# nanoporetech/taiyaki

Measured on AMD Instinct MI355X. Metric: signal-chunks/sec (T=4000) flip-flop train step, higher is better.
Workload: dtype f32; 1 GPU; configs[1]: mLstm_flipflop r9.4.1 DNA, chunk_len=4000 (T=800 blocks), 128 chunks/GPU, size 256, HIP flip-flop CRF loss + logZ, gradient maxima/clipping, AdamW; config_id=2, model=mLstm_flipflop, global_batch=128, chunk_len=4000, launch=hipGraph replay of forward+loss and of AdamW, eager backward, hw_queues=4, conv=gemm, lstm=miopen, batches=pre-assembled, cycled from HBM, parallelism=dp1 (reads sharded; one flat RCCL gradient all-reduce after backward)

## Files before the change

taiyaki_amd/csrc/lstm_kernels.hip:

```cpp
#include "dispatch.h"
#include "ff_common.h"
#include "lstm_bwd_layout.h"
#include "rnn_common.h"

namespace tk {
namespace {

template <int U>
constexpr int threads_for() { return U == 48 ? 384 : U <= 32 ? 256 : 512; }
template <int H, int U>
constexpr int bwd_threads_for() { return U == 48 ? 2 * H : threads_for<U>(); }

template <int H, int C, int U, bool VL = false, bool SAVE = !VL>
__global__ __launch_bounds__(threads_for<U>(), 1) void lstm_fwd_kernel(const float *__restrict__ gx,
                                                                       const float *__restrict__ whh, int T, Cols cols,
                                                                       int reverse, int ngroups,
                                                                       float *__restrict__ y,
                                                                       float *__restrict__ gates,
                                                                       float *__restrict__ cell, u64 *hbuf,
                                                                       uint32_t *status,
                                                                       const int32_t *__restrict__ lengths) {
    constexpr int NT = threads_for<U>();
    const int N = cols.n, LD = cols.ld();
    constexpr int G = H / U;
    constexpr int KP = NT / U;
    constexpr int KS = H / KP;
    constexpr int NG = (H * C + NT - 1) / NT;
    static_assert(KS >= 1 && KP <= 64 && C <= KP, "lane (u, kp) inside one wave; one cell lane per (u, column)");
    constexpr int U4 = U / 4;
    constexpr int NQ = SAVE ? (6 * C * U4 + NT - 1) / NT : 1;
    static_assert(U % 4 == 0, "a row of the staging block is whole 16-byte chunks");
    __shared__ __attribute__((aligned(16))) float hs[2][H * C];
    __shared__ __attribute__((aligned(16))) float stg[SAVE ? 2 : 1][SAVE ? 6 * C * U : 4];
    __shared__ int give_up;

    int group, member;
    place(G, group, member);
    const int tid = threadIdx.x;
    const int j0 = member * U, n0 = group * C;
    const int u = tid / KP, kp = tid % KP;

    float w[4][KS];
#pragma unroll
    for (int g = 0; g < 4; ++g)
#pragma unroll
        for (int i = 0; i < KS; ++i) w[g][i] = whh[((size_t)g * H + j0 + u) * H + i * KP + kp];
    settle(w);

    int col = 0;
#pragma unroll
    for (int m = 1, width = C; width > 1; m <<= 1, width >>= 1)
        if (kp & m) col += width / 2;
    const bool cell_lane = kp < C;
    const int n = n0 + col;
    const bool valid = cell_lane && n < N;
    float cst = 0.f;
    int len = 0;
    if constexpr (VL) len = !valid ? 0 : lengths ? lengths[n] : T;

    for (int i = tid; i < H * C; i += NT) hs[0][i] = 0.f;
    if (tid == 0) give_up = 0;

    const size_t H4 = 4 * (size_t)H;
    float *rp[NQ];
    size_t rpitch[NQ];
    if constexpr (SAVE) {
#pragma unroll
        for (int i = 0; i < NQ; ++i) {
            const int q = tid + i * NT, row = q / U4, v = row / C, nn = n0 + row % C;
            const size_t w = v < 2 ? (size_t)H : H4;
            float *base = v == 0 ? y : v == 1 ? cell : gates + (size_t)(v - 2) * H;
            rpitch[i] = (size_t)LD * w;
            rp[i] = q < 6 * C * U4 && nn < N ? base + (size_t)nn * w + j0 + 4 * (q % U4) : nullptr;
        }
    }
    float gq[4] = {0.f, 0.f, 0.f, 0.f};
    if (valid) {
        const float *p = gx + ((size_t)(reverse ? T - 1 : 0) * LD + n) * H4 + j0 + u;
#pragma unroll
        for (int g = 0; g < 4; ++g) gq[g] = p[(size_t)g * H];
    }
    float held = 0.f;
    __syncthreads();

    for (int s = 0; s < T; ++s) {
        const int t = reverse ? T - 1 - s : s;
        float *hb = hs[s & 1];
        settle(gq);
        if (s > 0) {
            const u64 *src = hbuf + ((size_t)((s - 1) & 1) * ngroups + group) * (H * C);
            float v[NG];
            if (!sweep<NG>(src, tid, NT, H * C, (unsigned)s, v, status)) give_up = 1;
#pragma unroll
            for (int q = 0; q < NG; ++q) {
                const int e = tid + q * NT;
                if (e < H * C) hb[(e % H) * C + e / H] = v[q];
            }
            __syncthreads();
            if (give_up) return;
            const int tl = reverse ? t + 1 : t - 1;
            if constexpr (!SAVE) {
                if (valid) y[((size_t)tl * LD + n) * H + j0 + u] = held;
            } else {
                rows_to_global<NQ>(stg[(s - 1) & 1], tid, NT, rp, rpitch, (size_t)tl);
            }
        }
        float gn[4] = {0.f, 0.f, 0.f, 0.f};
        if (valid && s + 1 < T) {
            const float *p = gx + ((size_t)(reverse ? t - 1 : t + 1) * LD + n) * H4 + j0 + u;
#pragma unroll
            for (int g = 0; g < 4; ++g) gn[g] = p[(size_t)g * H];
        }
        asm volatile("" ::: "memory");

        float acc[4][C];
#pragma unroll
        for (int g = 0; g < 4; ++g)
#pragma unroll
            for (int c = 0; c < C; ++c) acc[g][c] = 0.f;
#pragma unroll
        for (int i = 0; i < KS; ++i) {
            float hv[C];
            lds_row<C>(hb + (i * KP + kp) * C, hv);
#pragma unroll
            for (int g = 0; g < 4; ++g)
#pragma unroll
                for (int c = 0; c < C; ++c) acc[g][c] = fmaf(w[g][i], hv[c], acc[g][c]);
        }
#pragma unroll
        for (int m = 1; m < KP; m <<= 1) {
            const int half = C / (2 * m);
            const bool up = (kp & m) != 0;
#pragma unroll
            for (int g = 0; g < 4; ++g) {
                if (half == 0) acc[g][0] += __shfl_xor(acc[g][0], m);
#pragma unroll
                for (int c = 0; c < C / 2; ++c) {
                    if (c < half) {
                        const float send = up ? acc[g][c] : acc[g][c + half];
                        const float keep = up ? acc[g][c + half] : acc[g][c];
                        acc[g][c] = keep + __shfl_xor(send, m);
                    }
                }
            }
        }

        if (cell_lane) {
            float ig = sigmoidf(acc[0][0] + gq[0]), fg = sigmoidf(acc[1][0] + gq[1]);
            float gg = tanhf(acc[2][0] + gq[2]), og = sigmoidf(acc[3][0] + gq[3]);
            cst = fmaf(ig, gg, fg * cst);
            float h = og * tanhf(cst);
            if constexpr (VL) {
                if (t >= len) {
                    cst = h = 0.f;
                    if constexpr (SAVE) ig = fg = gg = og = 0.f;
                }
            }
            if (s + 1 < T)
                store_granule(hbuf + ((size_t)(s & 1) * ngroups + group) * (H * C) + col * H + j0 + u,
                              (unsigned)(s + 1), h);
            if constexpr (!SAVE) {
                held = h;
            } else {
                float *sp = stg[s & 1] + col * U + u;
                sp[0 * C * U] = h;
                sp[1 * C * U] = cst;
                sp[2 * C * U] = ig;
                sp[3 * C * U] = fg;
                sp[4 * C * U] = gg;
                sp[5 * C * U] = og;
            }
        }
#pragma unroll
        for (int g = 0; g < 4; ++g) gq[g] = gn[g];
    }
    if (T > 0) {
        const int tl = reverse ? 0 : T - 1;
        if constexpr (!SAVE) {
            if (valid) y[((size_t)tl * LD + n) * H + j0 + u] = held;
        } else {
            __syncthreads();
            rows_to_global<NQ>(stg[(T - 1) & 1], tid, NT, rp, rpitch, (size_t)tl);
        }
    }
}

#ifndef TK_RNN_VARLEN
template <int M>
__device__ __forceinline__ float xor_lane(float v) {
    static_assert(M == 1 || M == 2 || M == 4, "a partner inside the lane's group of 8");
    const int x = __float_as_int(v);
    if constexpr (M == 1) {
        return __int_as_float(__builtin_amdgcn_update_dpp(0, x, 0xB1, 0xF, 0xF, true));
    } else if constexpr (M == 2) {
        return __int_as_float(__builtin_amdgcn_update_dpp(0, x, 0x4E, 0xF, 0xF, true));
    } else {
        const int y = __builtin_amdgcn_update_dpp(0, x, 0x141, 0xF, 0xF, true);
        return __int_as_float(__builtin_amdgcn_update_dpp(0, y, 0x1B, 0xF, 0xF, true));
    }
}

template <int M, int RQ, int NA>
__device__ __forceinline__ void halve_rounds(float (&acc)[NA], int rq) {
    if constexpr (M < RQ) {
        constexpr int n = NA / (2 * M);
        const bool up = (rq & M) != 0;
#pragma unroll
        for (int a = 0; a < n; ++a) {
            const float send = up ? acc[a] : acc[a + n];
            const float keep = up ? acc[a + n] : acc[a];
            acc[a] = keep + xor_lane<M>(send);
        }
        halve_rounds<2 * M, RQ>(acc, rq);
    }
}

template <int H, int C, int U, bool VL = false>
__global__ __launch_bounds__((bwd_threads_for<H, U>()), 1) void lstm_bwd_kernel(const float *__restrict__ whh,
                                                                       const float *__restrict__ gates,
                                                                       const float *__restrict__ cell,
                                                                       const float *__restrict__ dy, int T, Cols cols,
                                                                       int reverse, int ngroups,
                                                                       float *__restrict__ dgates, u64 *pbuf,
                                                                       uint32_t *status,
                                                                       const int32_t *__restrict__ lengths) {
    constexpr int NT = bwd_threads_for<H, U>();
    const int N = cols.n, LD = cols.ld();
    constexpr int G = H / U;
    constexpr bool STRIDED = U == 48;
    constexpr int RP = NT / H;
    constexpr int R = 4 * U / RP;
    constexpr LstmBwdBlock LB(NT, H, U, C);
    constexpr bool BLOCK = LB.KQ > 0;
    constexpr int KQ = BLOCK ? LB.KQ : 1, RQ = BLOCK ? LB.RQ : 1, RR = BLOCK ? LB.RR : 1, KEEP = BLOCK ? LB.KEEP : 1;
    constexpr int PAIRS = U * C;
    constexpr int PL = NT / PAIRS;
    constexpr int NP = (G + PL - 1) / PL;
    constexpr bool APART = BLOCK && NP > 1;
    static_assert(!APART || NP * PL == G, "every plane polls NP producers");
    static_assert(RP >= 1 && R >= 1 && PL >= 1 && PL * PAIRS == NT, "every lane polls; one cell lane per pair");
    static_assert(!STRIDED || (RP * H == NT && R * RP == 4 * U && U % RP == 0),
                  "a lane's rows keep their gate index at compile time");
    static_assert(!BLOCK || (LB.ok() && KQ * RR * NT == 4 * U * H && RQ <= 64 && (RQ & (RQ - 1)) == 0 &&
                             KEEP * NT == C * H && KQ * RR == R),
                  "every owned weight in one lane; the RQ partial sums inside one wave; one granule per held sum");
    __shared__ __attribute__((aligned(16))) float dgs[4 * U * C];
    __shared__ float gath[(APART ? G : PL) * PAIRS];
    __shared__ __attribute__((aligned(16))) float red[RP > 1 && !BLOCK ? RP * C * H : 1];
    __shared__ int give_up;

    int group, member;
    place(G, group, member);
    const int tid = threadIdx.x;
    const int j0 = member * U, n0 = group * C;

    const int k = tid % H, rp = tid / H;
    const int kb = tid / RQ, rq = tid % RQ;
    float w[R];
    if constexpr (BLOCK) {
#pragma unroll
        for (int j = 0; j < RR; ++j) {
            const int r = LB.row(rq, j);
#pragma unroll
            for (int q = 0; q < KQ; ++q) w[q * RR + j] = whh[((size_t)(r / U) * H + j0 + (r % U)) * H + KQ * kb + q];
        }
    } else if constexpr (STRIDED) {
        const float *wbase = whh + (size_t)(j0 + rp) * H + k;
#pragma unroll
        for (int i = 0; i < R; ++i) w[i] = wbase[(unsigned)((((i * RP) / U) * H + (i * RP) % U) * H)];
    } else {
#pragma unroll
        for (int i = 0; i < R; ++i) {
            const int r = rp * R + i;
            w[i] = whh[((size_t)(r / U) * H + j0 + (r % U)) * H + k];
        }
    }
    settle(w);

    const bool cell_lane = tid < PAIRS;
    const int pair = tid % PAIRS, plane = tid / PAIRS;
    const int cc = pair / U, u = pair % U;
    const int n = n0 + cc;
    const bool valid = cell_lane && n < N;
    float dc_next = 0.f, f_next = 0.f;
    int len = 0;
    if constexpr (VL) len = !valid ? 0 : lengths ? lengths[n] : T;
    if (tid == 0) give_up = 0;

    const size_t H4 = 4 * (size_t)H;
    float in[7] = {0.f, 0.f, 0.f, 0.f, 0.f, 0.f, 0.f};
    if (valid) {
        const int t = reverse ? 0 : T - 1;
        const size_t o = ((size_t)t * LD + n) * H + j0 + u;
        in[0] = dy[o];
        in[1] = cell[o];
        if (T > 1) in[2] = cell[((size_t)(reverse ? t + 1 : t - 1) * LD + n) * H + j0 + u];
        const float *gp = gates + ((size_t)t * LD + n) * H4 + j0 + u;
#pragma unroll
        for (int g = 0; g < 4; ++g) in[3 + g] = gp[(size_t)g * H];
    }
    float held[4] = {0.f, 0.f, 0.f, 0.f};
    __syncthreads();

    const u64 *mine = pbuf + (size_t)group * G * C * H + cc * H + j0 + u;
    const int a0 = LB.kept_first(rq), pub = (a0 % C) * H + KQ * kb + a0 / C;
    for (int s = 0; s < T; ++s) {
        const int tt = T - 1 - s;
        const int t = reverse ? T - 1 - tt : tt;
        const int tp = reverse ? t + 1 : t - 1;
        settle(in);
        float dhr = 0.f;
        if (s > 0) {
            float v[NP];
            const int nvalid = plane < G ? (G - plane + PL - 1) / PL : 0;
            const u64 *src = mine + (size_t)((s - 1) & 1) * ngroups * G * C * H;
            if (!sweep<NP>(src, plane * C * H, PL * C * H, G * C * H, (unsigned)s, v, status)) give_up = 1;
            if constexpr (APART) {
#pragma unroll
                for (int q = 0; q < NP; ++q) gath[(plane + q * PL) * PAIRS + pair] = v[q];
            } else {
                float sum = 0.f;
#pragma unroll
                for (int q = 0; q < NP; ++q)
                    if (q < nvalid) sum += v[q];
                gath[plane * PAIRS + pair] = sum;
            }
            __syncthreads();
            if (give_up) return;
            if (cell_lane) {
#pragma unroll
                for (int p = 0; p < (APART ? G : PL); ++p) dhr += gath[p * PAIRS + pair];
            }
            if (valid) {
                const int tl = reverse ? t - 1 : t + 1;
                float *dp = dgates + ((size_t)tl * LD + n) * H4 + j0 + u;
#pragma unroll
                for (int g = 0; g < 4; ++g) dp[(size_t)g * H] = held[g];
            }
        }
        float nx[7] = {0.f, 0.f, 0.f, 0.f, 0.f, 0.f, 0.f};
        if (valid && tt > 0) {
            const size_t o = ((size_t)tp * LD + n) * H + j0 + u;
            nx[0] = dy[o];
            nx[1] = in[2];
            if (tt > 1) nx[2] = cell[((size_t)(reverse ? tp + 1 : tp - 1) * LD + n) * H + j0 + u];
            const float *gp = gates + ((size_t)tp * LD + n) * H4 + j0 + u;
#pragma unroll
            for (int g = 0; g < 4; ++g) nx[3 + g] = gp[(size_t)g * H];
        }
        asm volatile("" ::: "memory");

        if (cell_lane) {
            const float ct = in[1];
            float cp = in[2];
            if constexpr (VL) {
                if (tp >= len) cp = 0.f;
            }
            const float ig = in[3], gg = in[5], og = in[6];
            float fg = in[4];
            const float dh = in[0] + dhr;
            const float tc = tanhf(ct);
            float dc = dh * og * (1.f - tc * tc) + dc_next * f_next;
            float di = dc * gg * ig * (1.f - ig);
            float df = dc * cp * fg * (1.f - fg);
            float dg = dc * ig * (1.f - gg * gg);
            float dout = dh * tc * og * (1.f - og);
            if constexpr (VL) {
                if (t >= len) dc = fg = di = df = dg = dout = 0.f;
            }
            dc_next = dc;
            f_next = fg;
            held[0] = di;
            held[1] = df;
            held[2] = dg;
            held[3] = dout;
            dgs[(0 * U + u) * C + cc] = valid ? di : 0.f;
            dgs[(1 * U + u) * C + cc] = valid ? df : 0.f;
            dgs[(2 * U + u) * C + cc] = valid ? dg : 0.f;
            dgs[(3 * U + u) * C + cc] = valid ? dout : 0.f;
        }
#pragma unroll
        for (int q = 0; q < 7; ++q) in[q] = nx[q];
        __syncthreads();
        if (s + 1 == T) break;

        if constexpr (BLOCK) {
            u64 *dst = pbuf + (((size_t)(s & 1) * ngroups + group) * G + member) * C * H;
            float acc[KQ * C];
#pragma unroll
            for (int a = 0; a < KQ * C; ++a) acc[a] = 0.f;
#pragma unroll
            for (int i = 0; i < RR / 2; ++i) {
                float d[2 * C];
                lds_row<2 * C>(dgs + (rq + RQ * i) * 2 * C, d);
#pragma unroll
                for (int e = 0; e < 2; ++e)
#pragma unroll
                    for (int q = 0; q < KQ; ++q)
#pragma unroll
                        for (int c = 0; c < C; ++c)
                            acc[q * C + c] = fmaf(w[q * RR + 2 * i + e], d[e * C + c], acc[q * C + c]);
            }
            halve_rounds<1, RQ>(acc, rq);
#pragma unroll
            for (int v = 0; v < KEEP; ++v) store_granule(dst + pub + v * H, (unsigned)(s + 1), acc[v]);
            continue;
        }
        float acc[C];
#pragma unroll
        for (int c = 0; c < C; ++c) acc[c] = 0.f;
#pragma unroll
        for (int i = 0; i < R; ++i) {
            float d[C];
            lds_row<C>(dgs + (STRIDED ? i * RP + rp : rp * R + i) * C, d);
#pragma unroll
            for (int c = 0; c < C; ++c) acc[c] = fmaf(w[i], d[c], acc[c]);
        }
        u64 *dst = pbuf + (((size_t)(s & 1) * ngroups + group) * G + member) * C * H;
        if constexpr (RP == 1) {
#pragma unroll
            for (int c = 0; c < C; ++c) store_granule(dst + c * H + k, (unsigned)(s + 1), acc[c]);
        } else {
#pragma unroll
            for (int c = 0; c < C; ++c) red[(rp * C + c) * H + k] = acc[c];
            __syncthreads();
            for (int e = tid; e < C * H; e += NT) {
                float v = 0.f;
#pragma unroll
                for (int q = 0; q < RP; ++q) v += red[q * C * H + e];
                store_granule(dst + e, (unsigned)(s + 1), v);
            }
        }
    }
    if (valid && T > 0) {
        const int tl = reverse ? T - 1 : 0;
        float *dp = dgates + ((size_t)tl * LD + n) * H4 + j0 + u;
#pragma unroll
        for (int g = 0; g < 4; ++g) dp[(size_t)g * H] = held[g];
    }
}

#endif

int g_lab_cols = 0;
int g_lab_units = 0;

int units48(size_t H) { return H == 192 || H == 384 ? 48 : 0; }

bool lstm_geometry(size_t N, size_t H, int cu_count, int *C_out, int *groups_out) {
    const int U48 = units48(H);
    if (!(U48 || H == 16 || H == 32 || H == 64 || H == 128 || H == 256) || N == 0 || cu_count <= 0) return false;
    const size_t G = H / (U48 ? U48 : 16);
    const int first = U48 ? 4 : 8, last = H == 384 ? 4 : 2 * first;
    for (int C = first; C <= last; C *= 2) {
        if (g_lab_cols != 0 && C != g_lab_cols) continue;
        const size_t groups = (N + C - 1) / C;
        if (groups * G <= (size_t)cu_count) {
            *C_out = C;
            *groups_out = (int)groups;
            return true;
        }
    }
    return false;
}

size_t ws_bytes(size_t H, int C, int groups, int U, bool backward) {
    return 2 * (size_t)groups * (backward ? H / U : 1) * C * H * sizeof(u64);
}

struct Plan {
    int U, C, groups;
    unsigned grid;
};

bool lstm_plan(size_t N, size_t H, int cu_count, Plan *p) {
    int C16 = 0, groups16 = 0;
    if (!lstm_geometry(N, H, cu_count, &C16, &groups16)) return false;
    if (const int U48 = units48(H)) {
        *p = Plan{U48, C16, groups16, (unsigned)(groups16 * (H / U48))};
        return true;
    }
    int U = g_lab_units != 0 ? g_lab_units : 64;
    if ((size_t)U > H) U = (int)H;
    if (U != 16 && U != 32 && U != 64) return false;
    p->U = U;
    p->C = C16 * 16 / U;
    p->groups = (int)((N + p->C - 1) / p->C);
    p->grid = (unsigned)(p->groups * (H / U));
    return true;
}

#define TK_LSTM_SWITCH(LAUNCH)                                                                                    \
    switch ((int)H * 100000 + p.U * 1000 + p.C) {                                                                 \
        LAUNCH(16, 16, 8) LAUNCH(16, 16, 16) LAUNCH(32, 16, 8) LAUNCH(32, 16, 16) LAUNCH(64, 16, 8)                \
        LAUNCH(64, 16, 16) LAUNCH(128, 16, 8) LAUNCH(128, 16, 16) LAUNCH(256, 16, 8) LAUNCH(256, 16, 16)          \
        LAUNCH(32, 32, 4) LAUNCH(32, 32, 8) LAUNCH(64, 32, 4) LAUNCH(64, 32, 8) LAUNCH(128, 32, 4)                 \
        LAUNCH(128, 32, 8) LAUNCH(256, 32, 4) LAUNCH(256, 32, 8)                                                  \
        LAUNCH(64, 64, 2) LAUNCH(64, 64, 4) LAUNCH(128, 64, 2) LAUNCH(128, 64, 4) LAUNCH(256, 64, 2)               \
        LAUNCH(256, 64, 4) LAUNCH(192, 48, 4) LAUNCH(192, 48, 8) LAUNCH(384, 48, 4)                               \
        default: return TK_ERR_UNSUPPORTED;                                                                       \
    }

template <bool VL, bool SAVE>
int launch_fwd(const Plan &p, size_t H, hipStream_t st, const float *gx, const float *whh, int T, Cols cols,
               int rev, float *y, float *gates, float *cell, u64 *ws, uint32_t *status, const int32_t *lengths) {
#define TK_LSTM_FWD(HH, UU, CC)                                                                                  \
    case HH * 100000 + UU * 1000 + CC:                                                                           \
        hipLaunchKernelGGL((lstm_fwd_kernel<HH, CC, UU, VL, SAVE>), dim3(p.grid), dim3(threads_for<UU>()), 0, st, gx,  \
                           whh, T, cols, rev, p.groups, y, gates, cell, ws, status, lengths);                    \
        break;
    TK_LSTM_SWITCH(TK_LSTM_FWD)
#undef TK_LSTM_FWD
    return hipGetLastError() == hipSuccess ? TK_OK : TK_ERR_LAUNCH;
}

#ifndef TK_RNN_VARLEN
template <bool VL>
int launch_bwd(const Plan &p, size_t H, hipStream_t st, const float *whh, const float *gates, const float *cell,
               const float *dy, int T, Cols cols, int rev, float *dg, u64 *ws, uint32_t *status,
               const int32_t *lengths) {
#define TK_LSTM_BWD(HH, UU, CC)                                                                                   \
    case HH * 100000 + UU * 1000 + CC:                                                                            \
        hipLaunchKernelGGL((lstm_bwd_kernel<HH, CC, UU, VL>), dim3(p.grid), dim3(bwd_threads_for<HH, UU>()), 0,   \
                           st, whh, gates, cell, dy, T, cols, rev, p.groups, dg, ws, status, lengths);            \
        break;
    TK_LSTM_SWITCH(TK_LSTM_BWD)
#undef TK_LSTM_BWD
    return hipGetLastError() == hipSuccess ? TK_OK : TK_ERR_LAUNCH;
}
#endif
#undef TK_LSTM_SWITCH

size_t lstm_slab(size_t N, size_t H, int cu_count) {
    int C = 0, groups = 0;
    const size_t S = widest_admitted([&](size_t n) { return lstm_geometry(n, H, cu_count, &C, &groups); });
    return N == 0 ? 0 : N < S ? N : S;
}

template <class Launch>
int checked(bool pointers_ok, size_t T, size_t N, size_t H, int cu_count, void *ws, size_t wsb, uint32_t *status,
            hipStream_t stream, bool backward, Launch launch) {
    if (!pointers_ok || !ws || !status || !aligned16(ws) || T > (size_t)INT32_MAX || N > (size_t)INT32_MAX)
        return TK_ERR_BAD_ARG;
#ifdef TK_RNN_WIDE
    const size_t S = lstm_slab(N, H, cu_count);
#else
    const size_t S = N;
#endif
    if (S == 0) return TK_ERR_UNSUPPORTED;
    for (size_t first = 0; first < N; first += S) {
        const size_t n = N - first < S ? N - first : S;
        Plan p;
        if (!lstm_plan(n, H, cu_count, &p)) return TK_ERR_UNSUPPORTED;
        const size_t need = ws_bytes(H, p.C, p.groups, p.U, backward);
        if (wsb < need) return TK_ERR_WORKSPACE;
        if (T == 0) continue;
        int rc = zero_ws(ws, need, stream);
        if (rc != TK_OK) return rc;
        rc = launch(p, first, make_cols(n, N));
        if (rc != TK_OK) return rc;
    }
    return TK_OK;
}

size_t train_workspace_bytes(size_t N, size_t H, int cu_count) {
    int C = 0, groups = 0;
    if (!lstm_geometry(N, H, cu_count, &C, &groups)) return 0;
    const int U48 = units48(H);
    return ws_bytes(H, C, groups, U48 ? U48 : 16, true);
}

template <bool VL, bool SAVE>
int forward(const float *gx, const float *whh, const int32_t *lengths, size_t T, size_t N, size_t H, int reverse,
            int cu_count, float *y, float *gates, float *cell, void *ws, size_t wsb, uint32_t *status,
            hipStream_t stream) {
    auto launch = [&](const Plan &p, size_t first, Cols cols) {
        return launch_fwd<VL, SAVE>(p, H, stream, at_column(gx, first, 4 * H), whh, (int)T, cols, reverse,
                                    at_column(y, first, H), at_column(gates, first, 4 * H), at_column(cell, first, H),
                                    static_cast<u64 *>(ws), status, at_column(lengths, first, 1));
    };
    return checked(gx && whh && y && (!SAVE || (gates && cell)), T, N, H, cu_count, ws, wsb, status, stream, false,
                   launch);
}

#ifndef TK_RNN_VARLEN
template <bool VL>
int backward(const float *whh, const float *gates, const float *cell, const float *dy, const int32_t *lengths,
             size_t T, size_t N, size_t H, int reverse, int cu_count, float *dgates, void *ws, size_t wsb,
             uint32_t *status, hipStream_t stream) {
    auto launch = [&](const Plan &p, size_t first, Cols cols) {
        return launch_bwd<VL>(p, H, stream, whh, at_column(gates, first, 4 * H), at_column(cell, first, H),
                              at_column(dy, first, H), (int)T, cols, reverse, at_column(dgates, first, 4 * H),
                              static_cast<u64 *>(ws), status, at_column(lengths, first, 1));
    };
    return checked(whh && gates && cell && dy && dgates, T, N, H, cu_count, ws, wsb, status, stream, true, launch);
}
#endif

}

#ifdef TK_RNN_VARLEN
size_t lstm_varlen_workspace_bytes(size_t N, size_t H, int cu_count) {
    Plan p;
    if (!lstm_plan(N, H, cu_count, &p)) return 0;
    return ws_bytes(H, p.C, p.groups, p.U, false);
}

int lstm_forward_varlen_dispatch(const float *gx, const float *whh, const int32_t *lengths, size_t T, size_t N,
                                 size_t H, int reverse, int cu_count, float *y, void *ws, size_t wsb,
                                 uint32_t *status, hipStream_t stream) {
    return forward<true, false>(gx, whh, lengths, T, N, H, reverse, cu_count, y, nullptr, nullptr, ws, wsb, status,
                                stream);
}
#elif defined(TK_RNN_VARLEN_TRAIN)
size_t lstm_varlen_train_workspace_bytes(size_t N, size_t H, int cu_count) {
    return train_workspace_bytes(N, H, cu_count);
}

int lstm_forward_varlen_save_dispatch(const float *gx, const float *whh, const int32_t *lengths, size_t T, size_t N,
                                      size_t H, int reverse, int cu_count, float *y, float *gates, float *cell,
                                      void *ws, size_t wsb, uint32_t *status, hipStream_t stream) {
    return forward<true, true>(gx, whh, lengths, T, N, H, reverse, cu_count, y, gates, cell, ws, wsb, status, stream);
}

int lstm_backward_varlen_dispatch(const float *whh, const float *gates, const float *cell, const float *dy,
                                  const int32_t *lengths, size_t T, size_t N, size_t H, int reverse, int cu_count,
                                  float *dgates, void *ws, size_t wsb, uint32_t *status, hipStream_t stream) {
    return backward<true>(whh, gates, cell, dy, lengths, T, N, H, reverse, cu_count, dgates, ws, wsb, status, stream);
}
#elif defined(TK_RNN_WIDE)
size_t lstm_wide_slab(size_t N, size_t H, int cu_count) { return lstm_slab(N, H, cu_count); }

size_t lstm_wide_workspace_bytes(size_t N, size_t H, int cu_count) {
    return train_workspace_bytes(lstm_slab(N, H, cu_count), H, cu_count);
}

int lstm_forward_wide_dispatch(const float *gx, const float *whh, const int32_t *lengths, size_t T, size_t N,
                               size_t H, int reverse, int cu_count, float *y, float *gates, float *cell, void *ws,
                               size_t wsb, uint32_t *status, hipStream_t stream) {
    if (!gates != !cell) return TK_ERR_BAD_ARG;
    return gates ? forward<true, true>(gx, whh, lengths, T, N, H, reverse, cu_count, y, gates, cell, ws, wsb, status,
                                       stream)
                 : forward<true, false>(gx, whh, lengths, T, N, H, reverse, cu_count, y, nullptr, nullptr, ws, wsb,
                                        status, stream);
}

int lstm_backward_wide_dispatch(const float *whh, const float *gates, const float *cell, const float *dy,
                                const int32_t *lengths, size_t T, size_t N, size_t H, int reverse, int cu_count,
                                float *dgates, void *ws, size_t wsb, uint32_t *status, hipStream_t stream) {
    return backward<true>(whh, gates, cell, dy, lengths, T, N, H, reverse, cu_count, dgates, ws, wsb, status, stream);
}
#else
size_t lstm_workspace_bytes(size_t N, size_t H, int cu_count) { return train_workspace_bytes(N, H, cu_count); }

int lstm_forward_dispatch(const float *gx, const float *whh, size_t T, size_t N, size_t H, int reverse,
                          int cu_count, float *y, float *gates, float *cell, void *ws, size_t wsb,
                          uint32_t *status, hipStream_t stream) {
    return forward<false, true>(gx, whh, nullptr, T, N, H, reverse, cu_count, y, gates, cell, ws, wsb, status, stream);
}

int lstm_backward_dispatch(const float *whh, const float *gates, const float *cell, const float *dy, size_t T,
                           size_t N, size_t H, int reverse, int cu_count, float *dgates, void *ws, size_t wsb,
                           uint32_t *status, hipStream_t stream) {
    return backward<false>(whh, gates, cell, dy, nullptr, T, N, H, reverse, cu_count, dgates, ws, wsb, status, stream);
}

#ifdef TK_LAB
void lstm_lab_cols(int cols) { g_lab_cols = cols; }
void lstm_lab_units(int units) { g_lab_units = units; }

bool lstm_lab_geometry(size_t N, size_t H, int cu_count, size_t *out) {
    int C16 = 0, groups16 = 0;
    Plan p;
    if (!lstm_geometry(N, H, cu_count, &C16, &groups16) || !lstm_plan(N, H, cu_count, &p)) return false;
    const size_t v[8] = {(size_t)C16, (size_t)groups16, (size_t)p.U, (size_t)p.C, (size_t)p.groups, p.grid,
                         ws_bytes(H, p.C, p.groups, p.U, false), ws_bytes(H, p.C, p.groups, p.U, true)};
    for (int i = 0; i < 8; ++i) out[i] = v[i];
    return true;
}
#endif
#endif

}
```

Before: 5055 chunks/s.

## Add lane-split LSTM forward path reducing partial sums with DPP for H=256

Adds a specialised forward LSTM recurrence body for H=256, U=64, C=2. Each wave splits the k-dimension across 8 lanes, reduces the partial gate sums with DPP xor-halving rounds, and exchanges the four gate activations between lanes with DPP instead of shared memory. The hidden state is stored in shared memory in an interleaved layout so each lane reads whole 16-byte rows, with a prefetch distance of four rows. The goal is to shorten the per-timestep critical path of the serial recurrence. In exchange it adds a second code path with denser register use and relies on the DPP lane permutations matching the layout helpers.

After: 5307 chunks/s (median of 6 runs). 1.05x the previous value.

```diff
diff --git a/taiyaki_amd/csrc/lstm_fwd_layout.h b/taiyaki_amd/csrc/lstm_fwd_layout.h
--- /dev/null
+++ b/taiyaki_amd/csrc/lstm_fwd_layout.h
@@ -0,0 +1,42 @@
+#pragma once
+
+namespace tk {
+
+constexpr bool lstm_fwd_lanes(int H, int U, int C) { return H == 256 && U == 64 && C == 2; }
+
+struct LstmFwdLanes {
+    int NT, H, U, C;
+    int KP, KS, PR, CK;
+
+    constexpr LstmFwdLanes(int nt, int h, int u, int c)
+        : NT(nt), H(h), U(u), C(c), KP(nt / u), KS(h * u / nt), PR(c < 4 ? 4 / c : 1), CK(4 * c * u / nt) {}
+
+    constexpr bool ok() const {
+        return KP * U == NT && KS * KP == H && KP >= 4 && KP <= 64 && (KP & (KP - 1)) == 0 && PR >= 1 &&
+               (PR * C) % 4 == 0 && KS % PR == 0 && CK >= 1 && CK * KP == 4 * C && C % CK == 0;
+    }
+    constexpr int k(int kp, int i) const { return i * KP + kp; }
+    constexpr int hs_index(int k_, int c) const {
+        return ((k_ / KP / PR) * KP + k_ % KP) * PR * C + (k_ / KP % PR) * C + c;
+    }
+    constexpr int chunk(int kp, int j) const { return (j * KP + kp) * PR * C; }
+    constexpr int flat(int gate, int c) const { return (c / CK) * 4 * CK + gate * CK + c % CK; }
+    constexpr int kept_first(int kp) const {
+        int a = 0, n = 4 * C;
+        for (int m = 1; m < KP; m <<= 1) {
+            n /= 2;
+            if (kp & m) a += n;
+        }
+        return a;
+    }
+    constexpr int gate(int kp) const { return kept_first(kp) % (4 * CK) / CK; }
+    constexpr int col(int kp, int v) const { return kept_first(kp) / (4 * CK) * CK + v; }
+    constexpr bool cell_lane(int kp) const { return gate(kp) == 0; }
+    constexpr int gate_lane_xor(int g) const {
+        for (int x = 0; x < KP; ++x)
+            if (gate(x) == g && col(x, 0) == 0) return x;
+        return -1;
+    }
+};
+
+}
diff --git a/taiyaki_amd/csrc/lstm_kernels.hip b/taiyaki_amd/csrc/lstm_kernels.hip
--- a/taiyaki_amd/csrc/lstm_kernels.hip
+++ b/taiyaki_amd/csrc/lstm_kernels.hip
@@ -1,6 +1,7 @@
 #include "dispatch.h"
 #include "ff_common.h"
 #include "lstm_bwd_layout.h"
+#include "lstm_fwd_layout.h"
 #include "rnn_common.h"
 
 namespace tk {
@@ -10,6 +11,222 @@
 constexpr int threads_for() { return U == 48 ? 384 : U <= 32 ? 256 : 512; }
 template <int H, int U>
 constexpr int bwd_threads_for() { return U == 48 ? 2 * H : threads_for<U>(); }
+
+template <int M>
+__device__ __forceinline__ float xor_lane(float v) {
+    static_assert(M == 1 || M == 2 || M == 4, "a partner inside the lane's group of 8");
+    const int x = __float_as_int(v);
+    if constexpr (M == 1) {
+        return __int_as_float(__builtin_amdgcn_update_dpp(0, x, 0xB1, 0xF, 0xF, true));
+    } else if constexpr (M == 2) {
+        return __int_as_float(__builtin_amdgcn_update_dpp(0, x, 0x4E, 0xF, 0xF, true));
+    } else {
+        const int y = __builtin_amdgcn_update_dpp(0, x, 0x141, 0xF, 0xF, true);
+        return __int_as_float(__builtin_amdgcn_update_dpp(0, y, 0x1B, 0xF, 0xF, true));
+    }
+}
+
+template <int M, int RQ, int NA>
+__device__ __forceinline__ void halve_rounds(float (&acc)[NA], int rq) {
+    if constexpr (M < RQ) {
+        constexpr int n = NA / (2 * M);
+        const bool up = (rq & M) != 0;
+#pragma unroll
+        for (int a = 0; a < n; ++a) {
+            const float send = up ? acc[a] : acc[a + n];
+            const float keep = up ? acc[a + n] : acc[a];
+            acc[a] = keep + xor_lane<M>(send);
+        }
+        halve_rounds<2 * M, RQ>(acc, rq);
+    }
+}
+
+template <int H, int C, int U, bool VL, bool SAVE>
+__device__ __forceinline__ void lstm_fwd_lanes_body(const float *__restrict__ gx, const float *__restrict__ whh, int T,
+                                                    Cols cols, int reverse, int ngroups, float *__restrict__ y,
+                                                    float *__restrict__ gates, float *__restrict__ cell, u64 *hbuf,
+                                                    uint32_t *status, const int32_t *__restrict__ lengths) {
+    constexpr int NT = threads_for<U>();
+    const int N = cols.n, LD = cols.ld();
+    constexpr int G = H / U;
+    constexpr LstmFwdLanes FL(NT, H, U, C);
+    constexpr int KP = FL.KP, KS = FL.KS, PR = FL.PR, CK = FL.CK;
+    constexpr int NG = H * C / NT;
+    static_assert(FL.ok() && KP == 8 && NG * NT == H * C && FL.gate_lane_xor(1) == 4 && FL.gate_lane_xor(2) == 2 &&
+                      FL.gate_lane_xor(3) == 6,
+                  "whole rows in 16-byte reads; the partial sums and the four gates of a column inside 8 lanes of a wave");
+    constexpr int U4 = U / 4;
+    constexpr int NQ = SAVE ? (6 * C * U4 + NT - 1) / NT : 1;
+    static_assert(U % 4 == 0, "a row of the staging block is whole 16-byte chunks");
+    __shared__ __attribute__((aligned(16))) float hs[2][H * C];
+    __shared__ __attribute__((aligned(16))) float stg[SAVE ? 2 : 1][SAVE ? 6 * C * U : 4];
+    __shared__ int give_up;
+
+    int group, member;
+    place(G, group, member);
+    const int tid = threadIdx.x;
+    const int j0 = member * U, n0 = group * C;
+    const int u = tid / KP, kp = tid % KP;
+
+    float w[4][KS];
+#pragma unroll
+    for (int g = 0; g < 4; ++g)
+#pragma unroll
+        for (int i = 0; i < KS; ++i) w[g][i] = whh[((size_t)g * H + j0 + u) * H + FL.k(kp, i)];
+    settle(w);
+
+    const int gate = FL.gate(kp), col = FL.col(kp, 0);
+    const bool cell_lane = gate == 0;
+    const int n = n0 + col;
+    bool fetch[CK], valid[CK];
+    float cst[CK], held[CK];
+    int len[CK];
+#pragma unroll
+    for (int v = 0; v < CK; ++v) {
+        fetch[v] = n + v < N;
+        valid[v] = cell_lane && fetch[v];
+        cst[v] = held[v] = 0.f;
+        len[v] = 0;
+        if constexpr (VL) len[v] = !valid[v] ? 0 : lengths ? lengths[n + v] : T;
+    }
+
+    for (int i = tid; i < H * C; i += NT) hs[0][i] = 0.f;
+    if (tid == 0) give_up = 0;
+
+    const size_t H4 = 4 * (size_t)H;
+    float *rp[NQ];
+    size_t rpitch[NQ];
+    if constexpr (SAVE) {
+#pragma unroll
+        for (int i = 0; i < NQ; ++i) {
+            const int q = tid + i * NT, row = q / U4, v = row / C, nn = n0 + row % C;
+            const size_t w = v < 2 ? (size_t)H : H4;
+            float *base = v == 0 ? y : v == 1 ? cell : gates + (size_t)(v - 2) * H;
+            rpitch[i] = (size_t)LD * w;
+            rp[i] = q < 6 * C * U4 && nn < N ? base + (size_t)nn * w + j0 + 4 * (q % U4) : nullptr;
+        }
+    }
+    const float *gx0 = gx + (size_t)n * H4 + (size_t)gate * H + j0 + u;
+    float gq[CK];
+#pragma unroll
+    for (int v = 0; v < CK; ++v) gq[v] = fetch[v] ? gx0[(size_t)(reverse ? T - 1 : 0) * LD * H4 + v * H4] : 0.f;
+    __syncthreads();
+
+    for (int s = 0; s < T; ++s) {
+        const int t = reverse ? T - 1 - s : s;
+        float *hb = hs[s & 1];
+        settle(gq);
+        if (s > 0) {
+            const u64 *src = hbuf + ((size_t)((s - 1) & 1) * ngroups + group) * (H * C);
+            float v[NG];
+            if (!sweep<NG>(src, tid, NT, H * C, (unsigned)s, v, status)) give_up = 1;
+#pragma unroll
+            for (int q = 0; q < NG; ++q) {
+                const int e = tid + q * NT;
+                hb[FL.hs_index(e % H, e / H)] = v[q];
+            }
+            __syncthreads();
+            if (give_up) return;
+            const int tl = reverse ? t + 1 : t - 1;
+            if constexpr (!SAVE) {
+#pragma unroll
+                for (int v = 0; v < CK; ++v)
+                    if (valid[v]) y[((size_t)tl * LD + n + v) * H + j0 + u] = held[v];
+            } else {
+                rows_to_global<NQ>(stg[(s - 1) & 1], tid, NT, rp, rpitch, (size_t)tl);
+            }
+        }
+        float gn[CK];
+#pragma unroll
+        for (int v = 0; v < CK; ++v)
+            gn[v] = fetch[v] && s + 1 < T ? gx0[(size_t)(reverse ? t - 1 : t + 1) * LD * H4 + v * H4] : 0.f;
+        asm volatile("" ::: "memory");
+
+        float acc[4 * C];
+#pragma unroll
+        for (int a = 0; a < 4 * C; ++a) acc[a] = 0.f;
+        constexpr int NR = KS / PR, AHEAD = 4;
+        float hv[NR][PR * C];
+#pragma unroll
+        for (int j = 0; j < AHEAD; ++j) lds_row<PR * C>(hb + FL.chunk(kp, j), hv[j]);
+#pragma unroll
+        for (int j = 0; j < NR; ++j) {
+            if (j + AHEAD < NR) lds_row<PR * C>(hb + FL.chunk(kp, j + AHEAD), hv[j + AHEAD]);
+            __builtin_amdgcn_sched_barrier(0);
+#pragma unroll
+            for (int e = 0; e < PR; ++e)
+#pragma unroll
+                for (int g = 0; g < 4; ++g)
+#pragma unroll
+                    for (int c = 0; c < C; ++c)
+                        acc[FL.flat(g, c)] = fmaf(w[g][PR * j + e], hv[j][e * C + c], acc[FL.flat(g, c)]);
+        }
+        halve_rounds<1, KP>(acc, kp);
+
+        float ig[CK], fg[CK], gg[CK], og[CK];
+#pragma unroll
+        for (int v = 0; v < CK; ++v) {
+            const float x = acc[v] + gq[v];
+            float a;
+            if (gate == 2)
+                a = tanhf(x);
+            else
+                a = sigmoidf(x);
+            ig[v] = a;
+            gg[v] = xor_lane<2>(a);
+            fg[v] = xor_lane<4>(a);
+            og[v] = xor_lane<2>(fg[v]);
+        }
+
+        if (cell_lane) {
+            float h[CK];
+#pragma unroll
+            for (int v = 0; v < CK; ++v) {
+                cst[v] = fmaf(ig[v], gg[v], fg[v] * cst[v]);
+                h[v] = og[v] * tanhf(cst[v]);
+                if constexpr (VL) {
+                    if (t >= len[v]) {
+                        cst[v] = h[v] = 0.f;
+                        if constexpr (SAVE) ig[v] = fg[v] = gg[v] = og[v] = 0.f;
+                    }
+                }
+            }
+            if (s + 1 < T) {
+#pragma unroll
+                for (int v = 0; v < CK; ++v)
+                    store_granule(hbuf + ((size_t)(s & 1) * ngroups + group) * (H * C) + (col + v) * H + j0 + u,
+                                  (unsigned)(s + 1), h[v]);
+            }
+#pragma unroll
+            for (int v = 0; v < CK; ++v) {
+                if constexpr (!SAVE) {
+                    held[v] = h[v];
+                } else {
+                    float *sp = stg[s & 1] + (col + v) * U + u;
+                    sp[0 * C * U] = h[v];
+                    sp[1 * C * U] = cst[v];
+                    sp[2 * C * U] = ig[v];
+                    sp[3 * C * U] = fg[v];
+                    sp[4 * C * U] = gg[v];
+                    sp[5 * C * U] = og[v];
+                }
+            }
+        }
+#pragma unroll
+        for (int v = 0; v < CK; ++v) gq[v] = gn[v];
+    }
+    if (T > 0) {
+        const int tl = reverse ? 0 : T - 1;
+        if constexpr (!SAVE) {
+#pragma unroll
+            for (int v = 0; v < CK; ++v)
+                if (valid[v]) y[((size_t)tl * LD + n + v) * H + j0 + u] = held[v];
+        } else {
+            __syncthreads();
+            rows_to_global<NQ>(stg[(T - 1) & 1], tid, NT, rp, rpitch, (size_t)tl);
+        }
+    }
+}
 
 template <int H, int C, int U, bool VL = false, bool SAVE = !VL>
 __global__ __launch_bounds__(threads_for<U>(), 1) void lstm_fwd_kernel(const float *__restrict__ gx,
@@ -20,6 +237,10 @@
                                                                        float *__restrict__ cell, u64 *hbuf,
                                                                        uint32_t *status,
                                                                        const int32_t *__restrict__ lengths) {
+    if constexpr (lstm_fwd_lanes(H, U, C)) {
+        lstm_fwd_lanes_body<H, C, U, VL, SAVE>(gx, whh, T, cols, reverse, ngroups, y, gates, cell, hbuf, status, lengths);
+        return;
+    }
     constexpr int NT = threads_for<U>();
     const int N = cols.n, LD = cols.ld();
     constexpr int G = H / U;
@@ -186,35 +407,6 @@
 }
 
 #ifndef TK_RNN_VARLEN
-template <int M>
-__device__ __forceinline__ float xor_lane(float v) {
-    static_assert(M == 1 || M == 2 || M == 4, "a partner inside the lane's group of 8");
-    const int x = __float_as_int(v);
-    if constexpr (M == 1) {
-        return __int_as_float(__builtin_amdgcn_update_dpp(0, x, 0xB1, 0xF, 0xF, true));
-    } else if constexpr (M == 2) {
-        return __int_as_float(__builtin_amdgcn_update_dpp(0, x, 0x4E, 0xF, 0xF, true));
-    } else {
-        const int y = __builtin_amdgcn_update_dpp(0, x, 0x141, 0xF, 0xF, true);
-        return __int_as_float(__builtin_amdgcn_update_dpp(0, y, 0x1B, 0xF, 0xF, true));
-    }
-}
-
-template <int M, int RQ, int NA>
-__device__ __forceinline__ void halve_rounds(float (&acc)[NA], int rq) {
-    if constexpr (M < RQ) {
-        constexpr int n = NA / (2 * M);
-        const bool up = (rq & M) != 0;
-#pragma unroll
-        for (int a = 0; a < n; ++a) {
-            const float send = up ? acc[a] : acc[a + n];
-            const float keep = up ? acc[a + n] : acc[a];
-            acc[a] = keep + xor_lane<M>(send);
-        }
-        halve_rounds<2 * M, RQ>(acc, rq);
-    }
-}
-
 template <int H, int C, int U, bool VL = false>
 __global__ __launch_bounds__((bwd_threads_for<H, U>()), 1) void lstm_bwd_kernel(const float *__restrict__ whh,
                                                                        const float *__restrict__ gates,
```
